# zhb94430/RayTracer-Utah

Hardware: AMD Instinct MI355X
Metric: Mrays/sec at 1920x1080 (the reference's primary + secondary + shadow rays of the frames rendered / wall time; batched throughput: config.frames_in_flight frames with their own cameras per launch sequence — one frame alone: config.single_frame) (higher is better)
Workload: dtype f32

## Files before the change

include/rtu_render.h:

```cpp
#ifndef RTU_RENDER_H_INCLUDED
#define RTU_RENDER_H_INCLUDED

#include "rtu_scene.h"

#ifdef __cplusplus
extern "C" {
#endif

#define RTU_OK               0
#define RTU_ERR_ARG         (-1)
#define RTU_ERR_HIP         (-2)
#define RTU_ERR_UNSUPPORTED (-3)
#define RTU_ERR_STOCHASTIC  (-4)
#define RTU_ERR_NO_SCENE    (-5)
#define RTU_ERR_NO_DEVICE   (-6)
#define RTU_ERR_CAPACITY    (-7)
#define RTU_ERR_CANCELLED   (-8)
#define RTU_ERR_SCENE_SHAPE (-9)
#define RTU_ERR_STALE       (-10)

#define RTU_BAND_ROWS 8

typedef struct RtuContext RtuContext;

// ... 116 lines not shown

int  rtu_debug_node_bounds(RtuContext* ctx, int on);

int  rtu_debug_flags(RtuContext* ctx, uint32_t bits);
int  rtu_set_sequences_in_flight(RtuContext* ctx, int n);

int  rtu_debug_walk_stack_limit(RtuContext* ctx, uint32_t entries);

int  rtu_mesh_info(const RtuContext* ctx, uint32_t mesh, uint32_t* out5);

int  rtu_light_list_info(const RtuContext* ctx, uint32_t index, uint32_t* out5);

typedef struct RtuLightListDump {
    int32_t  usable, node, light;
    uint32_t G, point, n_entries;
    float    X[3], Y[3], Z[3], L[3], u0, v0, su, sv;
    uint32_t* cell_off;
    uint32_t* entry_face;
    float*    entry_zmin;
} RtuLightListDump;
int  rtu_debug_light_list(const RtuSceneDesc* scene, uint32_t light_slot, uint32_t cover_slot, RtuLightListDump* out);
void rtu_debug_light_list_free(RtuLightListDump* dump);
int  rtu_debug_context_light_list(RtuContext* ctx, uint32_t index, RtuLightListDump* out);
int  rtu_debug_update_timing(RtuContext* ctx, int on, float* ms_out5);

int  rtu_frame_counts(RtuContext* ctx, uint32_t* frames_out, uint32_t* deferred_out);

int  rtu_get_stats(RtuContext* ctx, RtuStats* stats);

#define RTU_KERNEL_SLOTS 40
typedef struct RtuTouched {
    uint64_t rays;
    uint64_t node_tests, mesh_box_tests, inner4, inner8, inner_ref, tri_tests, winners, xform_levels;
    uint64_t record_bytes;
    uint64_t bound_tests;
    uint64_t inline_shadow_rays;
} RtuTouched;
int         rtu_get_touched(RtuContext* ctx, RtuTouched* per_slot, int n_slots);
int         rtu_get_touched_launches(RtuContext* ctx, uint32_t* per_slot, int n_slots);
unsigned long long rtu_touched_bytes(const RtuTouched* t, int textured);
const char* rtu_kernel_slot_name(int slot);

int  rtu_probe_kernel(RtuContext* ctx, int slot);
int  rtu_probe_read(RtuContext* ctx, float* total_ms_out, int* launches_out);

int  rtu_time_render(RtuContext* ctx, const RtuFrameDesc* frame, void* d_rgbz, void* hip_stream,
// ... 37 lines not shown
```

raytracer-utah_amd/__init__.py:

```python
import ctypes
import os

_PKG = os.path.dirname(os.path.abspath(__file__))
_LIB = os.path.join(_PKG, "lib")

RTU_BIGFLOAT = 1.0e30
RTU_BAND_ROWS = 8

RTU_OK = 0
RTU_ERR_ARG = -1
RTU_ERR_HIP = -2
RTU_ERR_UNSUPPORTED = -3
RTU_ERR_STOCHASTIC = -4
RTU_ERR_NO_SCENE = -5
RTU_ERR_NO_DEVICE = -6
RTU_ERR_CAPACITY = -7
RTU_ERR_CANCELLED = -8
RTU_ERR_SCENE_SHAPE = -9
RTU_ERR_STALE = -10


class RtuError(RuntimeError):
    def __init__(self, code, msg=""):
        self.code = code
# ... 80 lines not shown
    path = os.path.join(_LIB, name)
    if not os.path.exists(path):
        raise ImportError("%s is missing: build the HIP extension first (__graft_entry__.build() or "
                          "`make -C raytracer-utah_amd`); there is no CPU fallback" % path)
    return ctypes.CDLL(path, mode=ctypes.RTLD_GLOBAL)


hip = _load("librtu_hip.so")
host = _load("librtu_host.so")

_P = ctypes.c_void_p
_I = ctypes.c_int


def _sig(lib, name, restype, *argtypes):
    fn = getattr(lib, name)
    fn.restype = restype
    fn.argtypes = list(argtypes)
    return fn


HIP_SYMBOLS = ["rtu_device_count", "rtu_error_string", "rtu_create_context", "rtu_destroy_context", "rtu_last_error",
               "rtu_upload_scene", "rtu_validate_scene", "rtu_frame_setup", "rtu_shard_rows", "rtu_shard_max_rows", "rtu_shard_global_row",
               "rtu_render_frame_device", "rtu_render_frames_device", "rtu_pack_image_device", "rtu_minmax_z_device", "rtu_pack_output_device", "rtu_render_frame", "rtu_frame_status", "rtu_render_timeline", "rtu_frame_counts", "rtu_timeline_exits", "rtu_mesh_info", "rtu_light_list_info", "rtu_debug_light_list", "rtu_update_scene", "rtu_multi_update_scene", "rtu_scene_shape_diff", "rtu_debug_context_light_list", "rtu_debug_update_timing", "rtu_debug_light_list_free", "rtu_debug_walk_stack_limit", "rtu_debug_node_bounds", "rtu_debug_flags", "rtu_set_sequences_in_flight", "rtu_debug_tail_from", "rtu_get_stats", "rtu_get_touched", "rtu_get_touched_launches", "rtu_touched_bytes", "rtu_kernel_slot_name", "rtu_probe_kernel", "rtu_probe_read", "rtu_time_render", "rtu_selftest_division", "rtu_selftest_primitives", "rtu_context_stream", "rtu_context_device", "rtu_context_sync", "rtu_host_alloc_pinned", "rtu_host_free_pinned", "rtu_copy_to_host_async", "rtu_device_alloc",
               "rtu_device_free", "rtu_copy_to_host", "rtu_device_info", "rtu_set_cancel_flag", "rtu_create_context_multi", "rtu_destroy_context_multi",
               "rtu_multi_size", "rtu_multi_context", "rtu_multi_last_error", "rtu_multi_upload_scene", "rtu_multi_render_frame", "rtu_multi_gather_kind",
               "rtu_adaptive_defaults", "rtu_render_frame_adaptive", "rtu_render_frame_adaptive_device", "rtu_debug_sample_images", "rtu_debug_texcoords",
               "rtu_debug_device_allocations", "rtu_progressive_begin", "rtu_progressive_advance", "rtu_progressive_status",
               "rtu_progressive_snapshot_device", "rtu_progressive_snapshot", "rtu_progressive_free", "rtu_debug_device_bytes"]
_sig(hip, "rtu_device_count", _I)
_sig(hip, "rtu_error_string", ctypes.c_char_p, _I)
_sig(hip, "rtu_create_context", _P, _I, ctypes.POINTER(_I))
_sig(hip, "rtu_destroy_context", None, _P)
_sig(hip, "rtu_last_error", ctypes.c_char_p, _P)
_sig(hip, "rtu_upload_scene", _I, _P, _P)
_sig(hip, "rtu_validate_scene", _I, _P, ctypes.c_char_p, ctypes.c_size_t)
_sig(hip, "rtu_frame_setup", _I, ctypes.POINTER(RtuCamera), _I, _I, ctypes.POINTER(RtuFrameDesc))
_sig(hip, "rtu_shard_rows", _I, ctypes.POINTER(RtuFrameDesc))
_sig(hip, "rtu_shard_max_rows", _I, _I, _I)
_sig(hip, "rtu_shard_global_row", _I, ctypes.POINTER(RtuFrameDesc), _I)
_sig(hip, "rtu_render_frame_device", _I, _P, ctypes.POINTER(RtuFrameDesc), _P, _P)
_sig(hip, "rtu_render_frames_device", _I, _P, ctypes.POINTER(RtuFrameDesc), _I, _P, _P)
_sig(hip, "rtu_pack_image_device", _I, _P, _P, ctypes.c_size_t, _P, _P, _P)
_sig(hip, "rtu_minmax_z_device", _I, _P, _P, ctypes.c_size_t, _I, _P, _P)
_sig(hip, "rtu_pack_output_device", _I, _P, _P, ctypes.c_size_t, _I, _P, _P, _P)
_sig(hip, "rtu_render_frame", _I, _P, ctypes.POINTER(RtuFrameDesc), _P, ctypes.POINTER(RtuStats))
_sig(hip, "rtu_frame_status", _I, _P)
# ... 74 lines not shown
_sig(hip, "rtu_destroy_context_multi", None, _P)
_sig(hip, "rtu_multi_size", _I, _P)
_sig(hip, "rtu_multi_context", _P, _P, _I)
_sig(hip, "rtu_multi_last_error", ctypes.c_char_p, _P)
_sig(hip, "rtu_multi_upload_scene", _I, _P, _P)
_sig(hip, "rtu_multi_render_frame", _I, _P, ctypes.POINTER(RtuFrameDesc), _P, ctypes.POINTER(RtuProgress))
_sig(hip, "rtu_multi_gather_kind", _I, _P)


class RtuLightListDump(ctypes.Structure):
    _fields_ = [("usable", ctypes.c_int32), ("node", ctypes.c_int32), ("light", ctypes.c_int32), ("G", ctypes.c_uint32), ("point", ctypes.c_uint32),
                ("n_entries", ctypes.c_uint32), ("X", ctypes.c_float * 3), ("Y", ctypes.c_float * 3), ("Z", ctypes.c_float * 3), ("L", ctypes.c_float * 3),
                ("u0", ctypes.c_float), ("v0", ctypes.c_float), ("su", ctypes.c_float), ("sv", ctypes.c_float),
                ("cell_off", ctypes.POINTER(ctypes.c_uint32)), ("entry_face", ctypes.POINTER(ctypes.c_uint32)), ("entry_zmin", ctypes.POINTER(ctypes.c_float))]


_sig(hip, "rtu_debug_light_list", _I, _P, ctypes.c_uint32, ctypes.c_uint32, ctypes.POINTER(RtuLightListDump))
_sig(hip, "rtu_debug_light_list_free", None, ctypes.POINTER(RtuLightListDump))
_sig(hip, "rtu_update_scene", _I, _P, _P)
_sig(hip, "rtu_multi_update_scene", _I, _P, _P)
_sig(hip, "rtu_scene_shape_diff", _I, _P, _P, ctypes.c_char_p, ctypes.c_size_t)
_sig(hip, "rtu_debug_context_light_list", _I, _P, ctypes.c_uint32, ctypes.POINTER(RtuLightListDump))
_sig(hip, "rtu_debug_update_timing", _I, _P, _I, ctypes.POINTER(ctypes.c_float))


def scene_shape_diff(a, b):
    buf = ctypes.create_string_buffer(256)
    rc = hip.rtu_scene_shape_diff(a.desc_ptr, b.desc_ptr, buf, len(buf))
    if rc == RTU_OK:
        return None
    if rc != RTU_ERR_SCENE_SHAPE:
        raise RtuError(rc, buf.value.decode())
    return buf.value.decode()


def _dump_dict(d):
    import numpy as np
    if not d.usable:
        return None
    n = d.G * d.G + 1
    return {"G": d.G, "point": bool(d.point), "X": np.array(list(d.X)), "Y": np.array(list(d.Y)), "Z": np.array(list(d.Z)), "L": np.array(list(d.L)),
            "u0": d.u0, "v0": d.v0, "su": d.su, "sv": d.sv, "node": d.node, "light": d.light,
            "cell_off": np.ctypeslib.as_array(d.cell_off, (n,)).copy(), "entry_face": np.ctypeslib.as_array(d.entry_face, (max(d.n_entries, 1),))[:d.n_entries].copy(),
            "entry_zmin": np.ctypeslib.as_array(d.entry_zmin, (max(d.n_entries, 1),))[:d.n_entries].copy()}


# ... 578 lines not shown
```

raytracer-utah_amd/csrc/render_impl.h:

```cpp
#ifndef RTU_RENDER_IMPL_H_INCLUDED
#define RTU_RENDER_IMPL_H_INCLUDED
#include "rtu_intersect.h"

namespace {

#define TEXD ((TEX & 1) != 0)
#define SMPD ((TEX & 2) != 0)
#define BATD ((TEX & 4) != 0)
#define GID ((TEX & 8) != 0)
#define CNTD ((TEX & 16) != 0)
#ifndef RTU_OCC_PRIMARY
#define RTU_OCC_PRIMARY __attribute__((amdgpu_waves_per_eu(4, 4)))
#endif
#ifndef RTU_OCC_PRIMARY_S
#define RTU_OCC_PRIMARY_S __attribute__((amdgpu_waves_per_eu(5, 5)))
#endif
#ifndef RTU_OCC_TRACE
#define RTU_OCC_TRACE __attribute__((amdgpu_waves_per_eu(5, 5)))
#endif
#ifndef RTU_OCC_WALK
#define RTU_OCC_WALK __attribute__((amdgpu_waves_per_eu(3, 3)))
#endif
#ifndef RTU_OCC_CONSUME
#define RTU_OCC_CONSUME
// ... 81 lines not shown
                         cnt.inner, cnt.leafv, cnt.leafe, cnt.tri, cnt.acc};
#pragma unroll
    for (int i = 0; i < 11; i++) {
        unsigned v = vals[i];
#pragma unroll
        for (int off = 32; off > 0; off >>= 1) v += __shfl_xor(v, off);
        if (lane_id() == 0 && v) atomicAdd(&a.counters[i], (unsigned long long)v);
    }
}
template <int TEX>
__device__ __forceinline__ void flush_touched(const KernelArgs& a, const Counters& cnt, int kid) {
    if (!CNTD) return;
    unsigned vals[RTU_TOUCH_FIELDS] = {cnt.t_rays, cnt.t_node, cnt.t_meshbox, cnt.t_inner4, cnt.t_inner8, cnt.t_innerref, cnt.t_tri, cnt.t_win,
                                       cnt.t_xform, cnt.t_bytes, cnt.t_bounds, cnt.t_inline};
#pragma unroll
    for (int i = 0; i < RTU_TOUCH_FIELDS; i++) {
        unsigned v = vals[i];
#pragma unroll
        for (int off = 32; off > 0; off >>= 1) v += __shfl_xor(v, off);
        if (lane_id() == 0 && v) atomicAdd(&a.counters[(size_t)kid * RTU_TOUCH_STRIDE + i], (unsigned long long)v);
    }
}

template <int TEX>
__device__ __forceinline__ uint32_t make_info(const KernelArgs& a, int mtl, int bounce, bool front, f3 dir, f3 p, f3 N, f3 uvw, Smp smp, bool amb = false) {
    const DevScene& s = a.scene;
    const RTU_CONST RtuMaterial& m = as_const(s.materials)[mtl];
    uint32_t info = (uint32_t)mtl | ((uint32_t)bounce << RTU_FI_BOUNCE_SH) | (front ? RTU_FI_FRONT : 0u);
    if (amb) info |= RTU_FI_AMB;
    else if (front && s.n_lights > 0) info |= RTU_FI_SH;
    if ((info & RTU_FI_SH) && s.nol_ok) {
        const uint32_t nl = a.nsl < RTU_FI_NOL_LIGHTS ? a.nsl : RTU_FI_NOL_LIGHTS;
        const float nn = dot3(N, N);
        for (uint32_t j = 0; j < nl; j++) {
            const f3 lvec = ld3(a.nol_light[j]);
            const f3 tl = a.nol_light[j][3] != 0.0f ? -lvec : lvec - p;
            const float c = dot3(N, tl), tt = dot3(tl, tl);
            if (c < 0.0f && c * c > 1e-6f * (tt * nn) && tt > 1e-20f && tt < 1e30f) info |= 1u << (RTU_FI_NOL_SH + j);
        }
    }
    if (bounce > 0) {
        if (not_black(mtl_color<TEXD>(s, mtl, RTU_MAP_REFRACTION, ld3(m.refraction), uvw))) {
            info |= RTU_FI_MAIN;
            Refr r = refraction_terms(dir, p, N, front, m.ior, smp, smp.on ? m.refraction_glossiness : 0.0f);
            if (r.sinTheta2 > 1) info |= RTU_FI_TIR;
        }
        if (not_black(mtl_color<TEXD>(s, mtl, RTU_MAP_REFLECTION, ld3(m.reflection), uvw))) info |= RTU_FI_C;
    }
    return info;
}

__device__ __forceinline__ f3 secondary_dir(int slot, uint32_t info, f3 dir, f3 p, f3 N, const RTU_CONST RtuMaterial& m, Smp smp) {
    if (slot == SLOT_C) return reflect_dir(dir, sampled_normal(p, N, smp, smp.on ? m.reflection_glossiness : 0.0f, RTU_DRAW_REFL));
    Refr t = refraction_terms(dir, p, N, (info & RTU_FI_FRONT) != 0, m.ior, smp, smp.on ? m.refraction_glossiness : 0.0f);
    if (info & RTU_FI_TIR) return reflect_dir(dir, t.sn);
    if (slot == SLOT_A) return reflect_dir(dir, t.sn2);
    return norm3((-t.sn2) * t.cosTheta2 + t.SVector * t.sinTheta2);
}

template <int TEX>
__device__ __forceinline__ uint32_t append_root(const KernelArgs& a, bool want, uint32_t shard, uint32_t info, f3 p, f3 N, uint32_t fbw, f3 dir,
// ... 225 lines not shown
        if (!deferred && leader) {
            if (!hit) {
                f3 bg = background_sample<TEXD>(s, x, y);
                if (!(a.dbg & 16u)) a.out[pix] = make_float4(bg.x, bg.y, bg.z, h.z);
                RTU_BYTES(16u);
            } else {
                RTU_CNT(prim_hit);
                mid = as_const(s.nodes)[h.node].material_id;
                if (mid < 0) { a.out[pix] = make_float4(1.0f, 1.0f, 1.0f, h.z); RTU_BYTES(16u); }
                else want = true;
            }
            if (GID) {
                a.gi_h[pix] = make_float4(h.p.x, h.p.y, h.p.z, h.z);
                a.gi_h[pix + a.gi_total] = make_float4(h.N.x, h.N.y, h.N.z, __uint_as_float((want ? 1u : 0u) | (h.front ? 2u : 0u) | ((uint32_t)(mid + 1) << 2)));
                a.gi_h[pix + 2u * (size_t)a.gi_total] = make_float4(ray.dir.x, ray.dir.y, ray.dir.z, __uint_as_float(smp.key));
                if (TEXD) a.gi_h[pix + 3u * (size_t)a.gi_total] = make_float4(h.uvw.x, h.uvw.y, h.uvw.z, 0.0f);
                RTU_BYTES(TEXD ? 64u : 48u);
                want = false;
            }
        }
    }
    if (GID) return;
    uint32_t info = 0;
    if (want) info = make_info<TEX>(a, mid, a.frame.max_bounce, h.front, ray.dir, h.p, h.N, h.uvw, smp);
    if (!STATS && INLINE_SHADE && !(a.dbg & 2048u) && __any(want && !(info & (RTU_FI_MAIN | RTU_FI_C)))) {
        const bool tryI = want && !(info & (RTU_FI_MAIN | RTU_FI_C));
        uint32_t lit = ~0u;
        bool ok = false;
        if (tryI) ok = shadows_inline<TEX>(a, info, h.p, lit, cnt);
        if (tryI && ok) {
            f3 direct = mk3(0, 0, 0);
            if (info & RTU_FI_SH) {
                const f3 cam_pos = BATD ? ld3(a.cam[sidx].pos) : ld3(a.frame.cam_pos);
                direct = direct_light<false, TEX>(a, info, h.p, h.N, h.uvw, cam_pos, direct, [&](uint32_t j) { return ((lit >> j) & 1u) ? 1.0f : 0.0f; });
            }
            a.out[pix] = make_float4(direct.x, direct.y, direct.z, h.z);
            RTU_BYTES(16u);
            want = false;
        }
    }
    if (!(a.dbg & 8u)) append_root<TEX>(a, want, shard, info, h.p, h.N, pix, ray.dir, h.z, h.uvw, cnt, !DEFER && !STATS);
    if (CNTD && !DEFER && !COOP && (a.dbg & 131072u) && valid) a.out[pix].x = (float)walk_units;
}

template <int STACK, bool STATS, int TEX>
__device__ __forceinline__ void primary_stage1(const KernelArgs& a, uint32_t n_tiles) {
    const Stamp stamp(a, RTU_TL_PRIMARY);
// ... 1210 lines not shown
```

raytracer-utah_amd/csrc/rtu_capi.hip:

```cpp
#include "rtu_devbuf.h"
#include "rtu_device.h"
#include "rtu_lightlist.h"

#include <algorithm>
#include <array>
#include <cmath>
#include <cstdarg>
#include <cstdio>
#include <cstdlib>
#include <cstring>
#include <map>
#include <memory>
#include <string>
#include <vector>

struct RtuProgressive;

struct RtuContext {
    int         device = 0;
    hipStream_t stream = nullptr;
    hipStream_t aux_stream = nullptr;
    hipEvent_t  aux_ev0 = nullptr, aux_ev1 = nullptr;
    hipEvent_t  ev0 = nullptr, ev1 = nullptr;
    std::string error;
// ... 91 lines not shown

int fail(RtuContext* ctx, int code, const char* fmt, ...) {
    char buf[512];
    va_list ap;
    va_start(ap, fmt);
    vsnprintf(buf, sizeof buf, fmt, ap);
    va_end(ap);
    if (ctx) ctx->error = buf;
    return code;
}

#define RTU_HIP(ctx, call)                                                                        \
    do {                                                                                          \
        hipError_t e_ = (call);                                                                   \
        if (e_ != hipSuccess) return fail(ctx, RTU_ERR_HIP, "%s: %s", #call, hipGetErrorString(e_)); \
    } while (0)

void free_scene(RtuContext* ctx) {
    ctx->scene_allocs.clear();
    ctx->place.clear();
    ctx->has_scene = false;
}

enum { P_NODES, P_MATERIALS, P_LIGHTS, P_MATMAPS, P_LMASK, P_COVER, P_LIST = P_COVER + RTU_MAX_COVER,
       P_SLOTS = P_LIST + 2 * RTU_LMASK_LIGHTS * RTU_MAX_COVER };

int ensure_place(RtuContext* ctx, int slot, size_t bytes, void** out) {
    if (ctx->place.size() < (size_t)P_SLOTS) ctx->place.resize(P_SLOTS);
    DevBuf<char>& b = ctx->place[(size_t)slot];
    RTU_HIP(ctx, b.grow(bytes ? bytes : 16));
    *out = b.get();
    return RTU_OK;
}

template <class T>
int place_upload(RtuContext* ctx, int slot, const T* src, size_t count, const T** dst) {
    void* d = nullptr;
    int rc = ensure_place(ctx, slot, sizeof(T) * count, &d);
    *dst = static_cast<const T*>(d);
    if (rc != RTU_OK) return rc;
    if (count) RTU_HIP(ctx, hipMemcpy(d, src, sizeof(T) * count, hipMemcpyHostToDevice));
    return RTU_OK;
}

template <class T>
int alloc_owned(RtuContext* ctx, std::vector<DevBuf<char>>& list, size_t bytes, T** dst) {
    list.emplace_back();
// ... 1388 lines not shown
    const hipStream_t streams[] = {ctx->aux_stream, ctx->stream};
    delete ctx;
    for (hipEvent_t e : events)
        if (e) (void)hipEventDestroy(e);
    for (hipStream_t s : streams)
        if (s) (void)hipStreamDestroy(s);
}

const char* rtu_last_error(const RtuContext* ctx) { return ctx ? ctx->error.c_str() : "context is NULL"; }

int rtu_validate_scene(const RtuSceneDesc* s, char* err_buf, size_t err_len) {
    RtuContext tmp;
    const int rc = validate(&tmp, s);
    if (err_buf && err_len) {
        snprintf(err_buf, err_len, "%s", tmp.error.c_str());
    }
    return rc;
}

}

namespace {

int place_scene(RtuContext* ctx, const RtuSceneDesc* s, bool on_device) {
    int rc;
    std::vector<DevNode> nodes(s->n_nodes);
    for (uint32_t i = 0; i < s->n_nodes; i++) {
        const RtuNode& n = s->nodes[i];
        DevNode& d = nodes[i];
        memset(&d, 0, sizeof d);
        memcpy(d.tm, n.tm, sizeof d.tm);
        memcpy(d.itm, n.itm, sizeof d.itm);
        memcpy(d.pos, n.pos, sizeof d.pos);
        d.parent = n.parent;
        d.obj_type = n.obj_type;
        d.mesh_id = n.mesh_id;
        d.material_id = n.material_id;
        d.depth = n.depth;
        int j = (int)i;
        for (int dd = n.depth; dd >= 0; dd--) {
            d.chain[dd] = j;
            j = s->nodes[j].parent;
        }
    }


// ... 55 lines not shown
    for (uint32_t i = 0; i < s->n_nodes && i < 64u; i++) {
        if (s->nodes[i].obj_type != RTU_OBJ_PLANE || ds.n_pcover >= RTU_MAX_PCOVER) continue;
        static const double sq[4][2] = {{-1, -1}, {1, -1}, {1, 1}, {-1, 1}};
        float quad[4][3];
        bool finite = true;
        for (int c = 0; c < 4; c++) {
            double p[3] = {sq[c][0], sq[c][1], 0.0};
            for (int j = (int)i; j >= 0; j = s->nodes[j].parent) {
                const RtuNode& t = s->nodes[j];
                const double q[3] = {p[0] * t.tm[0] + p[1] * t.tm[3] + p[2] * t.tm[6] + t.pos[0], p[0] * t.tm[1] + p[1] * t.tm[4] + p[2] * t.tm[7] + t.pos[1],
                                     p[0] * t.tm[2] + p[1] * t.tm[5] + p[2] * t.tm[8] + t.pos[2]};
                p[0] = q[0]; p[1] = q[1]; p[2] = q[2];
            }
            for (int k = 0; k < 3; k++) { quad[c][k] = (float)p[k]; finite = finite && std::isfinite(quad[c][k]); }
        }
        if (!finite) continue;
        ds.pcover_node[ds.n_pcover] = (int32_t)i;
        memcpy(ds.pcover_quad[ds.n_pcover], quad, sizeof quad);
        ds.n_pcover++;
    }
    ctx->light_list_info.clear();
    rc = on_device ? build_light_lists_device(ctx, s, cover_dev, lohi, wscale, ds) : build_light_lists(ctx, s, cover_host, wscale, ds);
    if (rc != RTU_OK) return rc;
    ds.obj_mask = 0;
    for (uint32_t i = 0; i < s->n_nodes && i < 64u; i++)
        if (s->nodes[i].obj_type != RTU_OBJ_NONE) ds.obj_mask |= 1ull << i;
    ds.n_lights = s->n_lights;
    env_value(s->background, ds.background);
    env_value(s->environment, ds.environment);
    ctx->dscene = ds;
    ctx->nsl = 0;
    for (uint32_t i = 0; i < s->n_lights; i++)
        if (s->lights[i].type != RTU_LIGHT_AMBIENT) {
            if (ctx->nsl < RTU_FI_NOL_LIGHTS) {
                for (int k = 0; k < 3; k++) ctx->nol_light[ctx->nsl][k] = s->lights[i].vec[k];
                ctx->nol_light[ctx->nsl][3] = s->lights[i].type == RTU_LIGHT_DIRECT ? 1.0f : 0.0f;
            }
            ctx->shadow_light[ctx->nsl++] = (int32_t)i;
        }
    memset(ctx->want_cap_s, 0, sizeof ctx->want_cap_s);
    ctx->want_defer_s = 0;
    ctx->tail_hint = 0;
    ctx->tail_hints.clear();
    ctx->list_hints.clear();
    ctx->mesh_hits_childless = true;
    for (uint32_t i = 0; i < s->n_nodes; i++) {
// ... 849 lines not shown
    make_cover_mesh(s, (uint32_t)node, sah.elements, cm);
    HostLightList hl;
    out->node = node;
    out->light = li;
    if (!compute_light_list(s->lights[li], cm, wscale, hl)) return RTU_OK;
    out->usable = 1;
    out->G = hl.m.G;
    out->point = hl.m.point;
    memcpy(out->X, hl.m.X, sizeof out->X); memcpy(out->Y, hl.m.Y, sizeof out->Y); memcpy(out->Z, hl.m.Z, sizeof out->Z); memcpy(out->L, hl.m.L, sizeof out->L);
    out->u0 = hl.m.u0; out->v0 = hl.m.v0; out->su = hl.m.su; out->sv = hl.m.sv;
    out->n_entries = (uint32_t)(hl.ent.size() / 2);
    out->cell_off = (uint32_t*)malloc(hl.off.size() * sizeof(uint32_t));
    out->entry_face = (uint32_t*)malloc((hl.ent.size() / 2 + 1) * sizeof(uint32_t));
    out->entry_zmin = (float*)malloc((hl.ent.size() / 2 + 1) * sizeof(float));
    if (!out->cell_off || !out->entry_face || !out->entry_zmin) { rtu_debug_light_list_free(out); return RTU_ERR_ARG; }
    memcpy(out->cell_off, hl.off.data(), hl.off.size() * sizeof(uint32_t));
    for (size_t e = 0; e < hl.ent.size() / 2; e++) {
        out->entry_face[e] = sah.elements[hl.ent[2 * e]];
        memcpy(&out->entry_zmin[e], &hl.ent[2 * e + 1], 4);
    }
    return RTU_OK;
}

void rtu_debug_light_list_free(RtuLightListDump* d) {
    if (!d) return;
    free(d->cell_off); free(d->entry_face); free(d->entry_zmin);
    d->cell_off = nullptr; d->entry_face = nullptr; d->entry_zmin = nullptr;
}

int rtu_debug_context_light_list(RtuContext* ctx, uint32_t index, RtuLightListDump* out) {
    if (!ctx || !out) return RTU_ERR_ARG;
    memset(out, 0, sizeof *out);
    if (!ctx->has_scene) return fail(ctx, RTU_ERR_NO_SCENE, "no scene uploaded");
    if (index >= ctx->light_list_info.size()) return fail(ctx, RTU_ERR_ARG, "no list %u", index);
    const RtuContext::LightListInfo& li = ctx->light_list_info[index];
    const uint32_t nc = ctx->dscene.n_cover;
    const DevLightMask& m = ctx->lmask_host[(size_t)li.light * nc + li.cover];
    const int node = ctx->dscene.cover_node[li.cover];
    const std::vector<uint32_t>& elements = ctx->fast_elements[(size_t)ctx->shape_nodes[(size_t)node].mesh_id];
    out->node = node;
    out->light = ctx->shadow_light[li.light];
    out->usable = 1;
    out->G = m.G;
    out->point = m.point;
    memcpy(out->X, m.X, sizeof out->X); memcpy(out->Y, m.Y, sizeof out->Y); memcpy(out->Z, m.Z, sizeof out->Z); memcpy(out->L, m.L, sizeof out->L);
    out->u0 = m.u0; out->v0 = m.v0; out->su = m.su; out->sv = m.sv;
// ... 178 lines not shown
```

raytracer-utah_amd/csrc/rtu_device.h:

```cpp
#ifndef RTU_DEVICE_H_INCLUDED
#define RTU_DEVICE_H_INCLUDED

#include "rtu_render.h"
#include "rtu_vec.h"

__device__ __forceinline__ int cvtt_i32(float v) { return (v > -2147483904.0f && v < 2147483648.0f) ? (int)v : (int)0x80000000; }

#define RTU_CONST __attribute__((address_space(4)))
template <class T> __device__ __forceinline__ const RTU_CONST T* as_const(const T* p) {
#pragma clang diagnostic push
#pragma clang diagnostic ignored "-Wold-style-cast"
    return (const RTU_CONST T*)(p);
#pragma clang diagnostic pop
}

#define RTU_GLOBAL __attribute__((address_space(1)))
typedef float rtu_v4f __attribute__((ext_vector_type(4)));
struct GBase {
    const RTU_GLOBAL char* p;
};
template <class T> __device__ __forceinline__ GBase global_base(const T* ptr) {
    const unsigned long long b = (unsigned long long)ptr;
    const unsigned lo = (unsigned)__builtin_amdgcn_readfirstlane((int)(unsigned)b), hi = (unsigned)__builtin_amdgcn_readfirstlane((int)(unsigned)(b >> 32));
    GBase g;
// ... 45 lines not shown
    const float4* bvh8;
    const float4* bvh4;
    uint32_t lds_nodes;
    uint32_t lds_off;
    float    scale;
};

#define RTU_MAX_PCOVER 8
struct DevNode {
    float   tm[9], itm[9], pos[3];
    int32_t parent, obj_type, mesh_id, material_id, depth;
    int32_t chain[RTU_MAX_NODE_DEPTH];
    float   wmin[3], wmax[3];
};

#define RTU_LMASK_LIGHTS 4u
#define RTU_LGRID_MAX 1024u
struct DevLightMask {
    float X[3], Y[3], Z[3], L[3];
    float u0, v0, su, sv;
    uint32_t usable, point, G, pad;
    const uint32_t* cell_off;
    const uint32_t* cell_tri;
};

struct DevTexture {
    int32_t type, width, height, pad;
    const uint8_t* rgb;
    float color1[3], color2[3];
};

struct DevScene {
    const DevNode*     nodes;
    const RtuMaterial* materials;
    const RtuLight*    lights;
    const DevMesh*     meshes;
    const DevTexture*  textures;
    const RtuTexMap*   mat_maps;
    RtuTexMap bg_map, env_map;
    RtuEnvColor bg, env;
    int32_t  img_w, img_h;
    uint32_t textured, pad_tex;
    uint32_t n_nodes, n_lights;
    uint32_t walk_stack_limit;
    float    wscale;
    unsigned long long obj_mask;
    uint32_t nol_ok, n_cover;
    int32_t  cover_node[8];
    const DevLightMask* lmask;
    const float4* cover_box[8];
    uint32_t cover_nf[8];
    uint32_t n_pcover, pad_pc;
    int32_t  pcover_node[RTU_MAX_PCOVER];
    float    pcover_quad[RTU_MAX_PCOVER][4][3];
    uint32_t dbg;
    uint32_t node_bounds;
    float    background[3];
    float    environment[3];
};

#define RTU_MAX_LEVELS        (RTU_MAX_BOUNCE + 1)
#define RTU_MAX_FRAME_BATCH 128
#define RTU_MAX_SHADOW_LIGHTS 13

#define RTU_FI_MTL_MASK   0x3FFFFu
#define RTU_FI_BOUNCE_SH  18
#define RTU_FI_FRONT      (1u << 21)
#define RTU_FI_SH         (1u << 22)
#define RTU_FI_MAIN       (1u << 23)
#define RTU_FI_TIR        (1u << 24)
#define RTU_FI_C          (1u << 25)
#define RTU_FI_NOL_SH     27
// ... 157 lines not shown
```

Baseline: 60820.

## Precompute conservative per-plane lit bitmaps to skip shadow rays on planes

```diff
diff --git a/include/rtu_render.h b/include/rtu_render.h
--- a/include/rtu_render.h
+++ b/include/rtu_render.h
@@ -162,6 +162,14 @@
 int  rtu_debug_light_list(const RtuSceneDesc* scene, uint32_t light_slot, uint32_t cover_slot, RtuLightListDump* out);
 void rtu_debug_light_list_free(RtuLightListDump* dump);
 int  rtu_debug_context_light_list(RtuContext* ctx, uint32_t index, RtuLightListDump* out);
+typedef struct RtuLitTableDump {
+    int32_t  usable, node, light;
+    uint32_t G;
+    float    O[3], U[3], V[3];
+    uint32_t* bits;
+} RtuLitTableDump;
+int  rtu_debug_lit_table(const RtuSceneDesc* scene, uint32_t node, uint32_t light_slot, RtuLitTableDump* out);
+void rtu_debug_lit_table_free(RtuLitTableDump* dump);
 int  rtu_debug_update_timing(RtuContext* ctx, int on, float* ms_out5);
 
 int  rtu_frame_counts(RtuContext* ctx, uint32_t* frames_out, uint32_t* deferred_out);
diff --git a/raytracer-utah_amd/__init__.py b/raytracer-utah_amd/__init__.py
--- a/raytracer-utah_amd/__init__.py
+++ b/raytracer-utah_amd/__init__.py
@@ -126,7 +126,7 @@
 
 HIP_SYMBOLS = ["rtu_device_count", "rtu_error_string", "rtu_create_context", "rtu_destroy_context", "rtu_last_error",
                "rtu_upload_scene", "rtu_validate_scene", "rtu_frame_setup", "rtu_shard_rows", "rtu_shard_max_rows", "rtu_shard_global_row",
-               "rtu_render_frame_device", "rtu_render_frames_device", "rtu_pack_image_device", "rtu_minmax_z_device", "rtu_pack_output_device", "rtu_render_frame", "rtu_frame_status", "rtu_render_timeline", "rtu_frame_counts", "rtu_timeline_exits", "rtu_mesh_info", "rtu_light_list_info", "rtu_debug_light_list", "rtu_update_scene", "rtu_multi_update_scene", "rtu_scene_shape_diff", "rtu_debug_context_light_list", "rtu_debug_update_timing", "rtu_debug_light_list_free", "rtu_debug_walk_stack_limit", "rtu_debug_node_bounds", "rtu_debug_flags", "rtu_set_sequences_in_flight", "rtu_debug_tail_from", "rtu_get_stats", "rtu_get_touched", "rtu_get_touched_launches", "rtu_touched_bytes", "rtu_kernel_slot_name", "rtu_probe_kernel", "rtu_probe_read", "rtu_time_render", "rtu_selftest_division", "rtu_selftest_primitives", "rtu_context_stream", "rtu_context_device", "rtu_context_sync", "rtu_host_alloc_pinned", "rtu_host_free_pinned", "rtu_copy_to_host_async", "rtu_device_alloc",
+               "rtu_render_frame_device", "rtu_render_frames_device", "rtu_pack_image_device", "rtu_minmax_z_device", "rtu_pack_output_device", "rtu_render_frame", "rtu_frame_status", "rtu_render_timeline", "rtu_frame_counts", "rtu_timeline_exits", "rtu_mesh_info", "rtu_light_list_info", "rtu_debug_light_list", "rtu_debug_lit_table", "rtu_debug_lit_table_free", "rtu_update_scene", "rtu_multi_update_scene", "rtu_scene_shape_diff", "rtu_debug_context_light_list", "rtu_debug_update_timing", "rtu_debug_light_list_free", "rtu_debug_walk_stack_limit", "rtu_debug_node_bounds", "rtu_debug_flags", "rtu_set_sequences_in_flight", "rtu_debug_tail_from", "rtu_get_stats", "rtu_get_touched", "rtu_get_touched_launches", "rtu_touched_bytes", "rtu_kernel_slot_name", "rtu_probe_kernel", "rtu_probe_read", "rtu_time_render", "rtu_selftest_division", "rtu_selftest_primitives", "rtu_context_stream", "rtu_context_device", "rtu_context_sync", "rtu_host_alloc_pinned", "rtu_host_free_pinned", "rtu_copy_to_host_async", "rtu_device_alloc",
                "rtu_device_free", "rtu_copy_to_host", "rtu_device_info", "rtu_set_cancel_flag", "rtu_create_context_multi", "rtu_destroy_context_multi",
                "rtu_multi_size", "rtu_multi_context", "rtu_multi_last_error", "rtu_multi_upload_scene", "rtu_multi_render_frame", "rtu_multi_gather_kind",
                "rtu_adaptive_defaults", "rtu_render_frame_adaptive", "rtu_render_frame_adaptive_device", "rtu_debug_sample_images", "rtu_debug_texcoords",
@@ -247,6 +247,32 @@
 _sig(hip, "rtu_scene_shape_diff", _I, _P, _P, ctypes.c_char_p, ctypes.c_size_t)
 _sig(hip, "rtu_debug_context_light_list", _I, _P, ctypes.c_uint32, ctypes.POINTER(RtuLightListDump))
 _sig(hip, "rtu_debug_update_timing", _I, _P, _I, ctypes.POINTER(ctypes.c_float))
+
+
+class RtuLitTableDump(ctypes.Structure):
+    _fields_ = [("usable", ctypes.c_int32), ("node", ctypes.c_int32), ("light", ctypes.c_int32), ("G", ctypes.c_uint32),
+                ("O", ctypes.c_float * 3), ("U", ctypes.c_float * 3), ("V", ctypes.c_float * 3), ("bits", ctypes.POINTER(ctypes.c_uint32))]
+
+
+_sig(hip, "rtu_debug_lit_table", _I, _P, ctypes.c_uint32, ctypes.c_uint32, ctypes.POINTER(RtuLitTableDump))
+_sig(hip, "rtu_debug_lit_table_free", None, ctypes.POINTER(RtuLitTableDump))
+
+
+def lit_table(scene, node, light_slot):
+    import numpy as np
+    d = RtuLitTableDump()
+    rc = hip.rtu_debug_lit_table(scene.desc_ptr, node, light_slot, ctypes.byref(d))
+    if rc != RTU_OK:
+        raise RtuError(rc, "rtu_debug_lit_table")
+    try:
+        if not d.usable:
+            return None
+        words = np.ctypeslib.as_array(d.bits, (d.G * d.G // 32,)).copy()
+        lit = np.unpackbits(words.view(np.uint8), bitorder="little").reshape(d.G, d.G).astype(bool)
+        return {"G": d.G, "O": np.array(list(d.O), np.float32), "U": np.array(list(d.U), np.float32), "V": np.array(list(d.V), np.float32),
+                "node": d.node, "light": d.light, "lit": lit}
+    finally:
+        hip.rtu_debug_lit_table_free(ctypes.byref(d))
 
 
 def scene_shape_diff(a, b):
diff --git a/raytracer-utah_amd/csrc/render_impl.h b/raytracer-utah_amd/csrc/render_impl.h
--- a/raytracer-utah_amd/csrc/render_impl.h
+++ b/raytracer-utah_amd/csrc/render_impl.h
@@ -127,8 +127,9 @@
     }
 }
 
-template <int TEX>
-__device__ __forceinline__ uint32_t make_info(const KernelArgs& a, int mtl, int bounce, bool front, f3 dir, f3 p, f3 N, f3 uvw, Smp smp, bool amb = false) {
+template <int TEX, bool LIT = false>
+__device__ __forceinline__ uint32_t make_info(const KernelArgs& a, int mtl, int bounce, bool front, f3 dir, f3 p, f3 N, f3 uvw, Smp smp, bool amb = false,
+                                              int node = -1) {
     const DevScene& s = a.scene;
     const RTU_CONST RtuMaterial& m = as_const(s.materials)[mtl];
     uint32_t info = (uint32_t)mtl | ((uint32_t)bounce << RTU_FI_BOUNCE_SH) | (front ? RTU_FI_FRONT : 0u);
@@ -142,6 +143,26 @@
             const f3 tl = a.nol_light[j][3] != 0.0f ? -lvec : lvec - p;
             const float c = dot3(N, tl), tt = dot3(tl, tl);
             if (c < 0.0f && c * c > 1e-6f * (tt * nn) && tt > 1e-20f && tt < 1e30f) info |= 1u << (RTU_FI_NOL_SH + j);
+        }
+    }
+    if (LIT && s.lit && !(a.dbg & 4096u)) {
+        const unsigned long long planes = as_const(s.lit)->planes;
+        const uint32_t nl = a.nsl < RTU_FI_NOL_LIGHTS ? a.nsl : RTU_FI_NOL_LIGHTS;
+        bool todo = (info & RTU_FI_SH) && node >= 0 && node < (int)RTU_LIT_NODES && ((planes >> (node & 63)) & 1ull);
+        while (__any(todo)) {
+            const int pn = __builtin_amdgcn_readlane(node, (int)__ffsll((long long)__ballot(todo)) - 1);
+            const bool mine = todo && node == pn;
+            for (uint32_t j = 0; j < nl; j++) {
+                const RTU_CONST DevLitTable& t = as_const(s.lit)->t[(uint32_t)pn * RTU_FI_NOL_LIGHTS + j];
+                if (!t.usable) continue;
+                const f3 d = p - ld3(t.O);
+                const float u = dot3(d, ld3(t.U)), v = dot3(d, ld3(t.V)), G = (float)t.G;
+                if (mine && !((info >> (RTU_FI_NOL_SH + j)) & 1u) && u >= 0.0f && v >= 0.0f && u < G && v < G) {
+                    const uint32_t cell = (uint32_t)v * t.G + (uint32_t)u;
+                    if ((t.bits[cell >> 5] >> (cell & 31u)) & 1u) info |= 1u << (RTU_FI_NOL_SH + j);
+                }
+            }
+            todo = todo && !mine;
         }
     }
     if (bounce > 0) {
@@ -413,7 +434,7 @@
     }
     if (GID) return;
     uint32_t info = 0;
-    if (want) info = make_info<TEX>(a, mid, a.frame.max_bounce, h.front, ray.dir, h.p, h.N, h.uvw, smp);
+    if (want) info = make_info<TEX, !STATS && !COOP>(a, mid, a.frame.max_bounce, h.front, ray.dir, h.p, h.N, h.uvw, smp, false, h.node);
     if (!STATS && INLINE_SHADE && !(a.dbg & 2048u) && __any(want && !(info & (RTU_FI_MAIN | RTU_FI_C)))) {
         const bool tryI = want && !(info & (RTU_FI_MAIN | RTU_FI_C));
         uint32_t lit = ~0u;
diff --git a/raytracer-utah_amd/csrc/rtu_capi.hip b/raytracer-utah_amd/csrc/rtu_capi.hip
--- a/raytracer-utah_amd/csrc/rtu_capi.hip
+++ b/raytracer-utah_amd/csrc/rtu_capi.hip
@@ -137,7 +137,7 @@
     ctx->has_scene = false;
 }
 
-enum { P_NODES, P_MATERIALS, P_LIGHTS, P_MATMAPS, P_LMASK, P_COVER, P_LIST = P_COVER + RTU_MAX_COVER,
+enum { P_NODES, P_MATERIALS, P_LIGHTS, P_MATMAPS, P_LMASK, P_LIT, P_LITBITS, P_COVER, P_LIST = P_COVER + RTU_MAX_COVER,
        P_SLOTS = P_LIST + 2 * RTU_LMASK_LIGHTS * RTU_MAX_COVER };
 
 int ensure_place(RtuContext* ctx, int slot, size_t bytes, void** out) {
@@ -1572,6 +1572,256 @@
 
 namespace {
 
+struct HostLitTable {
+    DevLitTable t;
+    std::vector<uint32_t> bits;
+};
+
+bool compute_lit_table(const RtuSceneDesc* s, const std::vector<DevNode>& nodes, float wscale, uint32_t P, const RtuLight& l, HostLitTable& out) {
+    memset(&out.t, 0, sizeof out.t);
+    out.bits.clear();
+    if (s->n_nodes > 64u || P >= RTU_LIT_NODES || s->nodes[P].obj_type != RTU_OBJ_PLANE) return false;
+    if (l.type != RTU_LIGHT_POINT && l.type != RTU_LIGHT_DIRECT) return false;
+    const bool point = l.type == RTU_LIGHT_POINT;
+    if (point && l.size > 0) return false;
+    if (!(wscale > 0) || !std::isfinite(wscale)) return false;
+    const uint32_t G = RTU_LIT_G;
+    double A[9] = {1, 0, 0, 0, 1, 0, 0, 0, 1}, b[3] = {0, 0, 0};
+    std::vector<int> chain;
+    for (int j = (int)P; j >= 0; j = s->nodes[j].parent) chain.push_back(j);
+    for (int j : chain) {
+        const RtuNode& n = s->nodes[j];
+        double M[9], nb[3];
+        for (int r = 0; r < 3; r++) {
+            for (int c = 0; c < 3; c++) M[3 * r + c] = n.tm[r] * A[c] + n.tm[3 + r] * A[3 + c] + n.tm[6 + r] * A[6 + c];
+            nb[r] = n.tm[r] * b[0] + n.tm[3 + r] * b[1] + n.tm[6 + r] * b[2] + n.pos[r];
+        }
+        memcpy(A, M, sizeof A); memcpy(b, nb, sizeof b);
+    }
+    const double det = A[0] * (A[4] * A[8] - A[5] * A[7]) - A[1] * (A[3] * A[8] - A[5] * A[6]) + A[2] * (A[3] * A[7] - A[4] * A[6]);
+    double nrm = 0;
+    for (int k = 0; k < 9; k++) nrm = std::max(nrm, std::fabs(A[k]));
+    if (!std::isfinite(det) || !(std::fabs(det) > 1e-12 * nrm * nrm * nrm)) return false;
+    const double Ti[9] = {(A[4] * A[8] - A[5] * A[7]) / det, (A[2] * A[7] - A[1] * A[8]) / det, (A[1] * A[5] - A[2] * A[4]) / det,
+                          (A[5] * A[6] - A[3] * A[8]) / det, (A[0] * A[8] - A[2] * A[6]) / det, (A[2] * A[3] - A[0] * A[5]) / det,
+                          (A[3] * A[7] - A[4] * A[6]) / det, (A[1] * A[6] - A[0] * A[7]) / det, (A[0] * A[4] - A[1] * A[3]) / det};
+    auto to_local = [&](const double w[3], double x[3]) {
+        const double d[3] = {w[0] - b[0], w[1] - b[1], w[2] - b[2]};
+        for (int r = 0; r < 3; r++) x[r] = Ti[3 * r] * d[0] + Ti[3 * r + 1] * d[1] + Ti[3 * r + 2] * d[2];
+    };
+    for (int k = 0; k < 9; k++) if (!std::isfinite(Ti[k])) return false;
+    double Ll[3];
+    const double lw[3] = {l.vec[0], l.vec[1], l.vec[2]};
+    if (point) to_local(lw, Ll);
+    else for (int r = 0; r < 3; r++) Ll[r] = -(Ti[3 * r] * lw[0] + Ti[3 * r + 1] * lw[1] + Ti[3 * r + 2] * lw[2]);
+    if (!(Ll[2] > 0) || !std::isfinite(Ll[0]) || !std::isfinite(Ll[1]) || !std::isfinite(Ll[2])) return false;
+    const double delta2 = 2e-4 * (double)wscale, W = 1e-4 * (double)wscale;
+    const double hz = delta2 * (std::fabs(Ti[6]) + std::fabs(Ti[7]) + std::fabs(Ti[8]));
+    const double cellw = 2.0 / G;
+    const double wx = cellw + W * (std::fabs(Ti[0]) + std::fabs(Ti[1]) + std::fabs(Ti[2])), wy = cellw + W * (std::fabs(Ti[3]) + std::fabs(Ti[4]) + std::fabs(Ti[5]));
+    out.bits.assign((size_t)G * G / 32, 0xFFFFFFFFu);
+    auto clear_rect = [&](double x0, double x1, double y0, double y1) {
+        const double c0 = std::floor((x0 - wx + 1.0) / cellw), c1 = std::floor((x1 + wx + 1.0) / cellw);
+        const double r0 = std::floor((y0 - wy + 1.0) / cellw), r1 = std::floor((y1 + wy + 1.0) / cellw);
+        if (!(c1 >= 0 && r1 >= 0 && c0 < (double)G && r0 < (double)G)) return;
+        const uint32_t ca = (uint32_t)std::max(c0, 0.0), cb = (uint32_t)std::min(c1, (double)G - 1), ra = (uint32_t)std::max(r0, 0.0), rb = (uint32_t)std::min(r1, (double)G - 1);
+        for (uint32_t r = ra; r <= rb; r++)
+            for (uint32_t c = ca; c <= cb; c++) out.bits[((size_t)r * G + c) >> 5] &= ~(1u << ((r * G + c) & 31u));
+    };
+    auto clear_hull = [&](std::vector<std::array<double, 2>>& pts, double x0, double x1, double y0, double y1) {
+        std::sort(pts.begin(), pts.end());
+        std::vector<std::array<double, 2>> h(2 * pts.size() + 2);
+        auto cross = [](const std::array<double, 2>& o, const std::array<double, 2>& a, const std::array<double, 2>& b) {
+            return (a[0] - o[0]) * (b[1] - o[1]) - (a[1] - o[1]) * (b[0] - o[0]);
+        };
+        size_t m = 0;
+        for (size_t i = 0; i < pts.size(); i++) { while (m >= 2 && cross(h[m - 2], h[m - 1], pts[i]) <= 0) m--; h[m++] = pts[i]; }
+        for (size_t i = pts.size() - 1, lo = m + 1; i-- > 0;) { while (m >= lo && cross(h[m - 2], h[m - 1], pts[i]) <= 0) m--; h[m++] = pts[i]; }
+        if (m < 4) { clear_rect(x0, x1, y0, y1); return; }
+        m--;
+        const double slack = 1e-9 * ((x1 - x0) + (y1 - y0) + 1.0) * ((x1 - x0) + (y1 - y0) + 1.0);
+        const double c0 = std::floor((x0 - wx + 1.0) / cellw), c1 = std::floor((x1 + wx + 1.0) / cellw);
+        const double r0 = std::floor((y0 - wy + 1.0) / cellw), r1 = std::floor((y1 + wy + 1.0) / cellw);
+        if (!(c1 >= 0 && r1 >= 0 && c0 < (double)G && r0 < (double)G)) return;
+        const uint32_t ca = (uint32_t)std::max(c0, 0.0), cb = (uint32_t)std::min(c1, (double)G - 1), ra = (uint32_t)std::max(r0, 0.0), rb = (uint32_t)std::min(r1, (double)G - 1);
+        for (uint32_t r = ra; r <= rb; r++)
+            for (uint32_t c = ca; c <= cb; c++) {
+                const double qx[2] = {-1.0 + cellw * c - wx, -1.0 + cellw * (c + 1) + wx}, qy[2] = {-1.0 + cellw * r - wy, -1.0 + cellw * (r + 1) + wy};
+                bool apart = false;
+                for (size_t e = 0; e < m && !apart; e++) {
+                    bool out = true;
+                    for (int q = 0; q < 4 && out; q++) out = cross(h[e], h[e + 1], {qx[q & 1], qy[q >> 1]}) < -slack;
+                    apart = out;
+                }
+                if (!apart) out.bits[((size_t)r * G + c) >> 5] &= ~(1u << ((r * G + c) & 31u));
+            }
+    };
+    for (uint32_t k = 0; k < s->n_nodes; k++) {
+        if (k == P || s->nodes[k].obj_type == RTU_OBJ_NONE) continue;
+        const DevNode& n = nodes[k];
+        double lo[3], hi[3];
+        bool inside = point;
+        for (int a = 0; a < 3; a++) {
+            if (!std::isfinite(n.wmin[a]) || !std::isfinite(n.wmax[a])) return false;
+            lo[a] = (double)n.wmin[a] - delta2; hi[a] = (double)n.wmax[a] + delta2;
+            if (point && !(lw[a] >= lo[a] && lw[a] <= hi[a])) inside = false;
+        }
+        if (inside) return false;
+        double C[8][3];
+        for (int c = 0; c < 8; c++) {
+            const double w[3] = {(c & 1) ? hi[0] : lo[0], (c & 2) ? hi[1] : lo[1], (c & 4) ? hi[2] : lo[2]};
+            to_local(w, C[c]);
+            if (point && !(C[c][2] < Ll[2] - hz)) return false;
+        }
+        double x0 = 1e300, x1 = -1e300, y0 = 1e300, y1 = -1e300;
+        std::vector<std::array<double, 2>> pts;
+        auto project = [&](const double q[3]) {
+            double x, y;
+            if (point) { const double f = Ll[2] / (Ll[2] - q[2]); x = Ll[0] + (q[0] - Ll[0]) * f; y = Ll[1] + (q[1] - Ll[1]) * f; }
+            else { const double f = q[2] / Ll[2]; x = q[0] - Ll[0] * f; y = q[1] - Ll[1] * f; }
+            x0 = std::min(x0, x); x1 = std::max(x1, x); y0 = std::min(y0, y); y1 = std::max(y1, y);
+            pts.push_back({x, y});
+        };
+        for (int c = 0; c < 8; c++)
+            for (int a = 0; a < 3; a++) {
+                if (c & (1 << a)) continue;
+                const double *p0 = C[c], *p1 = C[c | (1 << a)];
+                if (p0[2] < 0 && p1[2] < 0) continue;
+                double e0[3] = {p0[0], p0[1], p0[2]}, e1[3] = {p1[0], p1[1], p1[2]};
+                if (p0[2] < 0 || p1[2] < 0) {
+                    const double f = p0[2] / (p0[2] - p1[2]);
+                    double* e = p0[2] < 0 ? e0 : e1;
+                    e[0] = p0[0] + (p1[0] - p0[0]) * f; e[1] = p0[1] + (p1[1] - p0[1]) * f; e[2] = 0;
+                }
+                project(e0); project(e1);
+            }
+        if (x1 < x0) continue;
+        if (!std::isfinite(x0) || !std::isfinite(x1) || !std::isfinite(y0) || !std::isfinite(y1)) return false;
+        clear_hull(pts, x0, x1, y0, y1);
+    }
+    const double u = std::ldexp(1.0, -24);
+    double dmax = 1.0;
+    if (!point) dmax = std::sqrt(lw[0] * lw[0] + lw[1] * lw[1] + lw[2] * lw[2]);
+    double mag[3] = {1, 1, 0}, err[3] = {0, 0, 0};
+    auto absmul = [](const float* m, const double v[3], double o[3]) {
+        for (int r = 0; r < 3; r++) o[r] = std::fabs((double)m[r]) * v[0] + std::fabs((double)m[3 + r]) * v[1] + std::fabs((double)m[6 + r]) * v[2];
+    };
+    for (int j : chain) {
+        const RtuNode& n = s->nodes[j];
+        double tm_mag[3], tm_err[3];
+        absmul(n.tm, mag, tm_mag); absmul(n.tm, err, tm_err);
+        for (int r = 0; r < 3; r++) {
+            err[r] = tm_err[r] + 8 * u * (tm_mag[r] + std::fabs((double)n.pos[r]));
+            mag[r] = tm_mag[r] + std::fabs((double)n.pos[r]);
+        }
+    }
+    double E[2];
+    for (int pass = 0; pass < 2; pass++) {
+        double m2[3], e2[3];
+        for (int r = 0; r < 3; r++) { m2[r] = mag[r] + (pass ? dmax : 0.0); e2[r] = err[r] + (pass ? u * m2[r] : 0.0); }
+        for (size_t i = chain.size(); i-- > 0;) {
+            const RtuNode& n = s->nodes[chain[i]];
+            double dm[3], de[3], om[3], oe[3];
+            for (int r = 0; r < 3; r++) { dm[r] = m2[r] + std::fabs((double)n.pos[r]); de[r] = e2[r] + u * dm[r]; }
+            absmul(n.itm, dm, om); absmul(n.itm, de, oe);
+            for (int r = 0; r < 3; r++) { m2[r] = om[r]; e2[r] = oe[r] + 8 * u * om[r]; }
+        }
+        E[pass] = e2[2];
+    }
+    {
+        double R[9], rb[3];
+        memcpy(R, A, sizeof R); memcpy(rb, b, sizeof rb);
+        for (size_t i = chain.size(); i-- > 0;) {
+            const RtuNode& n = s->nodes[chain[i]];
+            double M[9], nb[3];
+            const double d[3] = {rb[0] - n.pos[0], rb[1] - n.pos[1], rb[2] - n.pos[2]};
+            for (int r = 0; r < 3; r++) {
+                for (int c = 0; c < 3; c++) M[3 * r + c] = n.itm[r] * R[c] + n.itm[3 + r] * R[3 + c] + n.itm[6 + r] * R[6 + c];
+                nb[r] = n.itm[r] * d[0] + n.itm[3 + r] * d[1] + n.itm[6 + r] * d[2];
+            }
+            memcpy(R, M, sizeof R); memcpy(rb, nb, sizeof rb);
+        }
+        const double resid = std::fabs(R[6]) + std::fabs(R[7]) + std::fabs(rb[2]);
+        for (int k = 0; k < 9; k++) if (!(std::fabs(R[k] - ((k % 4) == 0 ? 1.0 : 0.0)) < 1e-3)) return false;
+        E[0] += resid; E[1] += resid;
+        double rows = 0;
+        for (int r = 0; r < 3; r++) rows = std::max(rows, std::fabs(Ti[3 * r]) + std::fabs(Ti[3 * r + 1]) + std::fabs(Ti[3 * r + 2]));
+        E[1] += (std::fabs(R[6]) + std::fabs(R[7]) + std::fabs(R[8] - 1.0)) * rows * dmax;
+    }
+    if (!std::isfinite(E[0]) || !std::isfinite(E[1])) return false;
+    const double Esum = 2 * (E[0] + E[1]);
+    uint32_t lit = 0;
+    if (!point) {
+        const double dz = Ll[2] - Esum;
+        if (!(dz > 0 && E[0] / dz <= 1e-4)) std::fill(out.bits.begin(), out.bits.end(), 0u);
+    } else {
+        for (uint32_t r = 0; r < G; r++)
+            for (uint32_t c = 0; c < G; c++) {
+                const size_t cell = (size_t)r * G + c;
+                if (!((out.bits[cell >> 5] >> (cell & 31u)) & 1u)) continue;
+                double far2 = 0;
+                for (int q = 0; q < 4; q++) {
+                    const double x = -1.0 + cellw * (c + (q & 1)) + ((q & 1) ? wx : -wx), y = -1.0 + cellw * (r + (q >> 1)) + ((q >> 1) ? wy : -wy);
+                    double d2 = 0;
+                    for (int a = 0; a < 3; a++) { const double w = A[3 * a] * x + A[3 * a + 1] * y + b[a] - lw[a]; d2 += w * w; }
+                    far2 = std::max(far2, d2);
+                }
+                const double dz = (Ll[2] - E[0]) / (std::sqrt(far2) * (1 + 1e-6) + W) - Esum;
+                if (!(dz > 0 && E[0] / dz <= 1e-4)) out.bits[cell >> 5] &= ~(1u << (cell & 31u));
+            }
+    }
+    for (uint32_t w : out.bits) lit += (uint32_t)__builtin_popcount(w);
+    for (int a = 0; a < 3; a++) {
+        out.t.O[a] = (float)(-A[3 * a] - A[3 * a + 1] + b[a]);
+        out.t.U[a] = (float)(Ti[a] / cellw);
+        out.t.V[a] = (float)(Ti[3 + a] / cellw);
+        if (!std::isfinite(out.t.O[a]) || !std::isfinite(out.t.U[a]) || !std::isfinite(out.t.V[a])) return false;
+    }
+    out.t.G = G;
+    out.t.usable = lit > 0 ? 1u : 0u;
+    return out.t.usable != 0;
+}
+
+int build_lit_tables(RtuContext* ctx, const RtuSceneDesc* s, const std::vector<DevNode>& nodes, float wscale, DevScene& ds) {
+    const uint32_t nn = s->n_nodes < RTU_LIT_NODES ? s->n_nodes : RTU_LIT_NODES;
+    const size_t words = (size_t)RTU_LIT_G * RTU_LIT_G / 32;
+    std::vector<char> rec(sizeof(DevLitTables) + sizeof(DevLitTable) * (size_t)nn * RTU_FI_NOL_LIGHTS, 0);
+    std::vector<HostLitTable> made;
+    std::vector<size_t> where;
+    unsigned long long planes = 0;
+    for (uint32_t P = 0; P < nn; P++) {
+        if (s->nodes[P].obj_type != RTU_OBJ_PLANE) continue;
+        uint32_t slot = 0;
+        for (uint32_t i = 0; i < s->n_lights && slot < RTU_FI_NOL_LIGHTS; i++) {
+            if (s->lights[i].type == RTU_LIGHT_AMBIENT) continue;
+            HostLitTable h;
+            if (compute_lit_table(s, nodes, wscale, P, s->lights[i], h)) {
+                planes |= 1ull << P;
+                where.push_back((size_t)P * RTU_FI_NOL_LIGHTS + slot);
+                made.push_back(std::move(h));
+            }
+            slot++;
+        }
+    }
+    ds.lit = nullptr;
+    if (made.empty()) return RTU_OK;
+    void* dbits = nullptr;
+    int rc = ensure_place(ctx, P_LITBITS, made.size() * words * sizeof(uint32_t), &dbits);
+    if (rc != RTU_OK) return rc;
+    DevLitTables* hdr = reinterpret_cast<DevLitTables*>(rec.data());
+    hdr->planes = planes;
+    for (size_t i = 0; i < made.size(); i++) {
+        uint32_t* d = static_cast<uint32_t*>(dbits) + i * words;
+        RTU_HIP(ctx, hipMemcpy(d, made[i].bits.data(), words * sizeof(uint32_t), hipMemcpyHostToDevice));
+        made[i].t.bits = d;
+        hdr->t[where[i]] = made[i].t;
+    }
+    const char* drec = nullptr;
+    if ((rc = place_upload(ctx, P_LIT, rec.data(), rec.size(), &drec)) != RTU_OK) return rc;
+    ds.lit = reinterpret_cast<const DevLitTables*>(drec);
+    return RTU_OK;
+}
+
 int place_scene(RtuContext* ctx, const RtuSceneDesc* s, bool on_device) {
     int rc;
     std::vector<DevNode> nodes(s->n_nodes);
@@ -1673,6 +1923,7 @@
     ctx->light_list_info.clear();
     rc = on_device ? build_light_lists_device(ctx, s, cover_dev, lohi, wscale, ds) : build_light_lists(ctx, s, cover_host, wscale, ds);
     if (rc != RTU_OK) return rc;
+    if ((rc = build_lit_tables(ctx, s, nodes, wscale, ds)) != RTU_OK) return rc;
     ds.obj_mask = 0;
     for (uint32_t i = 0; i < s->n_nodes && i < 64u; i++)
         if (s->nodes[i].obj_type != RTU_OBJ_NONE) ds.obj_mask |= 1ull << i;
@@ -2568,6 +2819,38 @@
     return RTU_OK;
 }
 
+int rtu_debug_lit_table(const RtuSceneDesc* s, uint32_t node, uint32_t light_slot, RtuLitTableDump* out) {
+    if (!out) return RTU_ERR_ARG;
+    memset(out, 0, sizeof *out);
+    RtuContext tmp;
+    int rc = validate(&tmp, s);
+    if (rc != RTU_OK) return rc;
+    int li = -1;
+    uint32_t seen = 0;
+    for (uint32_t i = 0; i < s->n_lights; i++)
+        if (s->lights[i].type != RTU_LIGHT_AMBIENT && seen++ == light_slot) { li = (int)i; break; }
+    if (li < 0 || light_slot >= RTU_FI_NOL_LIGHTS || node >= s->n_nodes) return RTU_ERR_ARG;
+    std::vector<DevNode> nodes(s->n_nodes);
+    const float wscale = world_bounds(s, nodes);
+    out->node = (int32_t)node;
+    out->light = li;
+    HostLitTable h;
+    if (!compute_lit_table(s, nodes, wscale, node, s->lights[li], h)) return RTU_OK;
+    out->usable = 1;
+    out->G = h.t.G;
+    memcpy(out->O, h.t.O, sizeof out->O); memcpy(out->U, h.t.U, sizeof out->U); memcpy(out->V, h.t.V, sizeof out->V);
+    out->bits = (uint32_t*)malloc(h.bits.size() * sizeof(uint32_t));
+    if (!out->bits) return RTU_ERR_ARG;
+    memcpy(out->bits, h.bits.data(), h.bits.size() * sizeof(uint32_t));
+    return RTU_OK;
+}
+
+void rtu_debug_lit_table_free(RtuLitTableDump* d) {
+    if (!d) return;
+    free(d->bits);
+    d->bits = nullptr;
+}
+
 void rtu_debug_light_list_free(RtuLightListDump* d) {
     if (!d) return;
     free(d->cell_off); free(d->entry_face); free(d->entry_zmin);
diff --git a/raytracer-utah_amd/csrc/rtu_device.h b/raytracer-utah_amd/csrc/rtu_device.h
--- a/raytracer-utah_amd/csrc/rtu_device.h
+++ b/raytracer-utah_amd/csrc/rtu_device.h
@@ -91,6 +91,22 @@
     uint32_t usable, point, G, pad;
     const uint32_t* cell_off;
     const uint32_t* cell_tri;
+};
+
+#ifndef RTU_LIT_G
+#define RTU_LIT_G 256u
+#endif
+#define RTU_LIT_NODES 64u
+struct DevLitTable {
+    float O[3], U[3], V[3];
+    uint32_t G, usable;
+    uint32_t pad;
+    const uint32_t* bits;
+};
+struct DevLitTables {
+    unsigned long long planes;
+    unsigned long long pad;
+    DevLitTable t[1];
 };
 
 struct DevTexture {
@@ -117,6 +133,7 @@
     uint32_t nol_ok, n_cover;
     int32_t  cover_node[8];
     const DevLightMask* lmask;
+    const DevLitTables* lit;
     const float4* cover_box[8];
     uint32_t cover_nf[8];
     uint32_t n_pcover, pad_pc;
```

Result: no change. 60680 (median of 5 runs) (-0.2%).
